# Mourtz/Photorealistic-Rendering-using-OpenCL

Hardware: AMD Instinct MI355X
Metric: Msamples/s (width x height x spp / s) at 1920x1080 (higher is better)
Workload: dtype f32

## Files before the change

photorealistic-rendering-using-opencl_amd/csrc/hip/pt_device.h:

```cpp
#pragma once
#include <hip/hip_runtime.h>

#include "prt_detmath.h"
#include "prt_types.h"
#include "pt_filter.h"
#include "pt_layout.h"

namespace prt {
namespace dev {

#define PT_EPS 1e-5f
#define PT_INF 2e1f
#define PT_PI 3.1415926535897932384626433832795f
#define PT_TWO_PI 6.283185307179586476925286766559f
#define PT_INV_PI 0.3183098861837906715377675267450f
#define PT_INV_TWO_PI 0.1591549430918953357688837633725f
#define PT_INV_FOUR_PI 0.0795774715459476678844418816863f

#ifdef PT_EMU
#define PT_DEV __host__ __device__ __forceinline__
#else
#define PT_DEV __device__ __forceinline__
#endif
#define PT_HD __host__ __device__ __forceinline__

#if defined(__HIP_DEVICE_COMPILE__)
#define PT_WAVE_ANY(p) __builtin_expect(__builtin_amdgcn_ballot_w64(p) != 0ull, 0)
#endif

#ifndef PT_RECIP_STEPS
#define PT_RECIP_STEPS 1
#endif
PT_HD float hw_recip(float x) {
#if defined(__HIP_DEVICE_COMPILE__)
    const unsigned e = (prt_f2u(x) >> 23) & 0xffu;
    float r = __builtin_amdgcn_rcpf(x);
    for (int k = 0; k < PT_RECIP_STEPS; ++k) r = __builtin_fmaf(__builtin_fmaf(-x, r, 1.0f), r, r);
    if (PT_WAVE_ANY(!(e - 2u < 251u))) r = 1.0f / x;
    return r;
#else
    return 1.0f / x;
#endif
}
PT_HD float hw_sqrt(float x) {
#if defined(__HIP_DEVICE_COMPILE__)
    const unsigned e = (prt_f2u(x) >> 23) & 0x1ffu;
    const float r = __builtin_amdgcn_rsqf(x);
    const float s0 = x * r, hh = 0.5f * r;
    float s = __builtin_fmaf(__builtin_fmaf(-s0, s0, x), hh, s0);
    if (PT_WAVE_ANY(!(e - 27u < 200u))) s = __builtin_sqrtf(x);
    return s;
#else
    return __builtin_sqrtf(x);
#endif
}
struct f3 { float x, y, z; };
PT_HD f3 F3(float x, float y, float z) { f3 r; r.x = x; r.y = y; r.z = z; return r; }
PT_HD f3 splat(float s) { return F3(s, s, s); }
PT_HD f3 operator+(f3 a, f3 b) { return F3(a.x + b.x, a.y + b.y, a.z + b.z); }
PT_HD f3 operator-(f3 a, f3 b) { return F3(a.x - b.x, a.y - b.y, a.z - b.z); }
PT_HD f3 operator*(f3 a, f3 b) { return F3(a.x * b.x, a.y * b.y, a.z * b.z); }
PT_HD f3 operator*(f3 a, float s) { return F3(a.x * s, a.y * s, a.z * s); }
PT_HD f3 operator/(f3 a, float s) { return F3(a.x / s, a.y / s, a.z / s); }
PT_HD f3 operator-(f3 a) { return F3(-a.x, -a.y, -a.z); }
PT_HD float dot(f3 a, f3 b) { return a.x * b.x + a.y * b.y + a.z * b.z; }
PT_HD f3 cross(f3 a, f3 b) { return F3(a.y * b.z - a.z * b.y, a.z * b.x - a.x * b.z, a.x * b.y - a.y * b.x); }
PT_HD float length(f3 a) { return hw_sqrt(a.x * a.x + a.y * a.y + a.z * a.z); }
PT_HD f3 normalize(f3 a) { float inv = hw_recip(hw_sqrt(a.x * a.x + a.y * a.y + a.z * a.z)); return F3(a.x * inv, a.y * inv, a.z * inv); }
PT_HD f3 ld3(const float* p) { return F3(p[0], p[1], p[2]); }

#if defined(__HIP_DEVICE_COMPILE__)
#define PT_CONST __attribute__((address_space(4)))
#else
#define PT_CONST
#endif
typedef float pt_vf4 __attribute__((ext_vector_type(4)));
typedef unsigned pt_vu4 __attribute__((ext_vector_type(4)));
template <typename T> PT_HD const PT_CONST pt_vf4* const_vf4(const T* p) { return (const PT_CONST pt_vf4*)p; }
PT_HD unsigned const_u32(const uint32_t* p, unsigned i) { return ((const PT_CONST uint32_t*)p)[i]; }
PT_HD int const_i32(const int32_t* p, unsigned i) { return ((const PT_CONST int32_t*)p)[i]; }
PT_HD float const_f32(const float* p, size_t i) { return ((const PT_CONST float*)p)[i]; }
template <typename T> PT_HD unsigned table_offset(unsigned i) {
    static_assert(sizeof(T) == 64 || sizeof(T) == 48, "NodePair, or a 48-byte record");
    return sizeof(T) == 64 ? pair_offset(i) : rec48_offset(i);
}
template <typename T> PT_HD const float4* table_at(const T* base, unsigned i) { return reinterpret_cast<const float4*>(reinterpret_cast<const char*>(base) + table_offset<T>(i)); }
template <typename T> PT_HD const PT_CONST pt_vf4* const_table_at(const T* base, unsigned i) { return (const PT_CONST pt_vf4*)((const PT_CONST char*)base + table_offset<T>(i)); }
template <typename T> PT_HD const PT_CONST pt_vf4* const_lane_at(const T* base, unsigned i) { return (const PT_CONST pt_vf4*)((const PT_CONST char*)base + i * (unsigned)sizeof(T)); }
PT_HD DevSphere sphere_of(const PT_CONST pt_vf4* q) {
    const pt_vf4 a = q[0];
    DevSphere s;
    s.pos[0] = a.x; s.pos[1] = a.y; s.pos[2] = a.z; s.radius = a.w;
    return s;
}
PT_HD DevSphere const_sphere(const DevSphere* p, unsigned i) { return sphere_of(const_vf4(p + i)); }
PT_HD DevSphere lane_sphere(const DevSphere* p, unsigned i) { return sphere_of(const_lane_at(p, i)); }
PT_HD DevQuad quad_of(const PT_CONST pt_vf4* q) {
    const pt_vf4 a = q[0], b = q[1], c = q[2], d = q[3], e = q[4];
    DevQuad r;
    r.base[0] = a.x; r.base[1] = a.y; r.base[2] = a.z; r.area = a.w;
    r.edge0[0] = b.x; r.edge0[1] = b.y; r.edge0[2] = b.z; r.e0e0 = b.w;
    r.edge1[0] = c.x; r.edge1[1] = c.y; r.edge1[2] = c.z; r.e1e1 = c.w;
    r.normal[0] = d.x; r.normal[1] = d.y; r.normal[2] = d.z; r.u0 = d.w;
    r.anchor[0] = e.x; r.anchor[1] = e.y; r.anchor[2] = e.z; r.u1 = e.w;
    return r;
}
PT_HD DevQuad const_quad(const DevQuad* p, unsigned i) { return quad_of(const_vf4(p + i)); }
PT_HD DevQuad lane_quad(const DevQuad* p, unsigned i) { return quad_of(const_lane_at(p, i)); }
PT_HD DevSdf sdf_of(const PT_CONST pt_vf4* q) {
    const pt_vf4 a = q[0], b = q[1];
    DevSdf r;
    r.pos[0] = a.x; r.pos[1] = a.y; r.pos[2] = a.z; r.type = prt_f2u(a.w);
    r.params[0] = b.x; r.params[1] = b.y; r.params[2] = b.z; r.params[3] = b.w;
    return r;
}
PT_HD DevSdf const_sdf(const DevSdf* p, unsigned i) { return sdf_of(const_vf4(p + i)); }
PT_HD DevSdf lane_sdf(const DevSdf* p, unsigned i) { return sdf_of(const_lane_at(p, i)); }
PT_DEV f3 vexp(f3 a) { return F3(prt_exp(a.x), prt_exp(a.y), prt_exp(a.z)); }
PT_DEV float fmax3(f3 v) { return prt_fmax(prt_fmax(v.x, v.y), v.z); }
PT_DEV float avg3(f3 v) { return (v.x * 1.0f + v.y * 1.0f + v.z * 1.0f) * 0.3333333333333333333333333333333333333333333333f; }

PT_DEV float hw_min(float a, float b) { return __builtin_fminf(a, b); }
PT_DEV float hw_max(float a, float b) { return __builtin_fmaxf(a, b); }

struct Rng { unsigned s0, s1; };
PT_DEV float next1D(Rng& r) {
    r.s0 = 36969u * (r.s0 & 65535u) + (r.s0 >> 16);
    r.s1 = 18000u * (r.s1 & 65535u) + (r.s1 >> 16);
    unsigned ires = (r.s0 << 16) + r.s1;
    return (prt_u2f((ires & 0x007fffffu) | 0x40000000u) - 2.0f) * 0.5f;
}

struct Frame { f3 normal, tangent, bitangent; };
PT_DEV Frame make_frame(f3 n) {
    Frame f;
    float sn = prt_copysign(1.0f, n.z);
    float a = -hw_recip(sn + n.z);
    float b = n.x * n.y * a;
    f.normal = n;
    f.tangent = F3(1.0f + sn * n.x * n.x * a, sn * b, -sn * n.x);
    f.bitangent = F3(b, sn + n.y * n.y * a, -n.y);
    return f;
}
PT_DEV f3 to_local(const Frame& f, f3 p) { return F3(dot(f.tangent, p), dot(f.bitangent, p), dot(f.normal, p)); }
PT_DEV f3 to_global(const Frame& f, f3 p) { return f.tangent * p.x + f.bitangent * p.y + f.normal * p.z; }

struct Ray {
    f3 origin, dir, normal, pos;
    float t;
    bool backside;
    float time;
};

struct Event {
    f3 wi, wo, weight;
    float pdf;
    unsigned sampledLobe;
    Frame frame;
};

struct Mat {
    f3 color, eta, k;
    float roughness;
    unsigned t, lobes, dist;
};
template <unsigned DM = 7u>
PT_DEV Mat load_mat(const DevMaterial* mats, unsigned i) {
    Mat r;
    const PT_CONST pt_vf4* q = const_table_at(mats, i);
    const pt_vf4 a = q[0], e = q[1], kk = q[2];
    r.color = F3(a.x, a.y, a.z); r.roughness = a.w;
    r.eta = F3(e.x, e.y, e.z); r.k = F3(kk.x, kk.y, kk.z);
    unsigned b = prt_f2u(e.w);
    r.t = b & 0xffffu; r.lobes = (b >> 16) & 0xffu; r.dist = (b >> 24) & DM;
    return r;
}

PT_DEV unsigned mat_bits(const DevMaterial* mats, unsigned i) { return *(const PT_CONST uint32_t*)((const PT_CONST char*)mats + (rec48_offset(i) + 28u)); }
PT_DEV unsigned mat_index(int mesh_id) { return (unsigned)(mesh_id + 1) & 0xffffffu; }

PT_DEV void sincos_pair(float x, float& sin_out, float& cos_out) {
    const bool unsupported = !(prt_fabs(x) < 1.0e9f);
    float s, c; int q;
    prt_sincos_kernel(unsupported ? 0.0f : x, &s, &c, &q);
    const float vs = (q & 1) ? c : s, vc = (q & 1) ? s : c;
    const float sn = (q & 2) ? -vs : vs, cs = ((q + 1) & 2) ? -vc : vc;
    const float z = x - x;
    sin_out = unsupported ? z : sn;
    cos_out = unsupported ? z : cs;
}

PT_DEV f3 uniform_sphere(float xi_x, float xi_y) {
    float phi = xi_x * PT_TWO_PI;
    float z = xi_y * 2.0f - 1.0f;
    float r = hw_sqrt(prt_fmax(1.0f - z * z, 0.0f));
    float sn, cs;
    sincos_pair(phi, sn, cs);
    return F3(cs * r, sn * r, z);
}
PT_DEV f3 cosine_hemisphere(float xi_x, float xi_y) {
    float phi = xi_x * PT_TWO_PI;
    float r = hw_sqrt(xi_y);
    float sn, cs;
    sincos_pair(phi, sn, cs);
    return F3(cs * r, sn * r, hw_sqrt(prt_fmax(1.0f - xi_y, 0.0f)));
}
PT_DEV bool check_reflection(f3 wi, f3 wo) {
    return prt_fabs(wi.z * wo.z - wi.x * wo.x - wi.y * wo.y - 1.0f) < 1e-3f;
}
PT_DEV bool check_refraction(f3 wi, f3 wo, float eta, float cosThetaT) {
    float dotP = -wi.x * wo.x * eta - wi.y * wo.y * eta - prt_copysign(cosThetaT, wi.z) * wo.z;
    return prt_fabs(dotP - 1.0f) < 1e-3f;
}

PT_HD void camera_basis(const prt_camera& in, DevCamera& cam) {
    f3 view = normalize(ld3(in.view));
    f3 up = normalize(ld3(in.up));
    f3 hAxis = normalize(cross(view, up));
    f3 vAxis = normalize(cross(hAxis, view));
    f3 position = ld3(in.position);
    f3 middle = position + view;
    f3 horizontal = hAxis * prt_tan(in.fov[0] * 0.5f * (PT_PI / 180));
    f3 vertical = vAxis * prt_tan(in.fov[1] * -0.5f * (PT_PI / 180));
    cam.position[0] = position.x; cam.position[1] = position.y; cam.position[2] = position.z;
    cam.hAxis[0] = hAxis.x; cam.hAxis[1] = hAxis.y; cam.hAxis[2] = hAxis.z;
    cam.vAxis[0] = vAxis.x; cam.vAxis[1] = vAxis.y; cam.vAxis[2] = vAxis.z;
    cam.middle[0] = middle.x; cam.middle[1] = middle.y; cam.middle[2] = middle.z;
    cam.horizontal[0] = horizontal.x; cam.horizontal[1] = horizontal.y; cam.horizontal[2] = horizontal.z;
    cam.vertical[0] = vertical.x; cam.vertical[1] = vertical.y; cam.vertical[2] = vertical.z;
    cam.apertureRadius = in.apertureRadius; cam.focalDistance = in.focalDistance;
}

PT_DEV Ray create_cam_ray(int cx, int cy, int width, int height, const DevCamera& cam, Rng& rng) {
    const f3 hAxis = ld3(cam.hAxis), vAxis = ld3(cam.vAxis), position = ld3(cam.position);
    const f3 middle = ld3(cam.middle), horizontal = ld3(cam.horizontal), vertical = ld3(cam.vertical);
    int pixelx = cx;
    int pixely = height - cy - 1;
    float sx = (float)pixelx / (width - 1.0f);
    float sy = (float)pixely / (height - 1.0f);
    f3 onPlane = middle + (horizontal * ((2 * sx) - 1)) + (vertical * ((2 * sy) - 1));
    f3 onImagePlane = position + ((onPlane - position) * cam.focalDistance);
    f3 aperturePoint;
    if (cam.apertureRadius > 0.00001f) {
        float random1 = next1D(rng);
        float random2 = next1D(rng);
        float angle = 2 * PT_PI * random1;
        float distance = cam.apertureRadius * hw_sqrt(random2);
        float sn, cs;
        sincos_pair(angle, sn, cs);
        float apertureX = cs * distance;
        float apertureY = sn * distance;
        aperturePoint = position + (hAxis * apertureX) + (vAxis * apertureY);
    } else {
        aperturePoint = position;
    }
    Ray ray;
    ray.backside = false;
    ray.origin = aperturePoint;
    ray.dir = normalize(onImagePlane - aperturePoint);
    ray.time = next1D(rng);
    ray.normal = splat(0.0f);
    ray.pos = splat(0.0f);
    ray.t = 0.0f;
    return ray;
}
PT_DEV Ray create_cam_ray_at(int cx, int cy, float dx, float dy, int width, int height, const DevCamera& cam, Rng& rng) {
    const f3 hAxis = ld3(cam.hAxis), vAxis = ld3(cam.vAxis), position = ld3(cam.position);
    const f3 middle = ld3(cam.middle), horizontal = ld3(cam.horizontal), vertical = ld3(cam.vertical);
    const int pixely = height - cy - 1;
    const float sx = ((float)cx + dx) / (width - 1.0f);
    const float sy = ((float)pixely - dy) / (height - 1.0f);
    const f3 onPlane = middle + (horizontal * ((2 * sx) - 1)) + (vertical * ((2 * sy) - 1));
    const f3 onImagePlane = position + ((onPlane - position) * cam.focalDistance);
    f3 aperturePoint;
    if (cam.apertureRadius > 0.00001f) {
        const float random1 = next1D(rng);
        const float random2 = next1D(rng);
        const float angle = 2 * PT_PI * random1;
        const float distance = cam.apertureRadius * hw_sqrt(random2);
        float sn, cs;
        sincos_pair(angle, sn, cs);
        const float apertureX = cs * distance;
        const float apertureY = sn * distance;
        aperturePoint = position + (hAxis * apertureX) + (vAxis * apertureY);
    } else {
        aperturePoint = position;
    }
    Ray ray;
    ray.backside = false;
    ray.origin = aperturePoint;
    ray.dir = normalize(onImagePlane - aperturePoint);
    ray.time = next1D(rng);
    ray.normal = splat(0.0f);
    ray.pos = splat(0.0f);
    ray.t = 0.0f;
    return ray;
}

struct RayPre { float ix, iy, iz, sx, sy, sz; bool nx, ny, nz; };
PT_DEV RayPre ray_pre(const Ray& ray) {
    RayPre p;
    p.ix = hw_recip(ray.dir.x); p.iy = hw_recip(ray.dir.y); p.iz = hw_recip(ray.dir.z);
    p.sx = -ray.origin.x * p.ix; p.sy = -ray.origin.y * p.iy; p.sz = -ray.origin.z * p.iz;
    p.nx = ray.dir.x < 0.0f; p.ny = ray.dir.y < 0.0f; p.nz = ray.dir.z < 0.0f;
    return p;
}

struct TriHit { float u, v; unsigned slot; };

PT_DEV bool hit_triangle_data(const float4 a, const float4 b, const float4 c4, const unsigned slot, const Ray& ray, float& best_t, TriHit& th) {
    const f3 p0 = F3(a.x, a.y, a.z), e1 = F3(a.w, b.x, b.y), e2 = F3(b.z, b.w, c4.x), n = F3(c4.y, c4.z, c4.w);
    f3 c = p0 - ray.origin;
    f3 r = cross(ray.dir, c);
    float inv_det = hw_recip(dot(n, ray.dir));
    float u = dot(r, e2) * inv_det;
    float v = dot(r, e1) * inv_det;
    float w = 1.0f - u - v;
    if (u >= 0 && v >= 0 && w >= 0) {
        float t = dot(n, c) * inv_det;
        if (t > PT_EPS && t < best_t) {
            best_t = t;
            th.u = u; th.v = v; th.slot = slot;
            return true;
        }
    }
    return false;
}
PT_DEV bool hit_triangle(const TriGeom* __restrict__ tg, unsigned slot, const Ray& ray, float& best_t, TriHit& th) {
    const PT_CONST pt_vf4* q = const_vf4(tg + slot);
    const pt_vf4 a = q[0], b = q[1], c4 = q[2];
    return hit_triangle_data(make_float4(a.x, a.y, a.z, a.w), make_float4(b.x, b.y, b.z, b.w), make_float4(c4.x, c4.y, c4.z, c4.w), slot, ray, best_t, th);
}

struct TravStack {
    unsigned* lds;
    unsigned stride;
};

struct PairData { float4 b0, b1, b2; uint4 meta; };
PT_DEV PairData load_pair(const NodePair* __restrict__ pairs, unsigned node) {
    const float4* q = table_at(pairs, node);
    PairData d;
    d.b0 = q[0]; d.b1 = q[1]; d.b2 = q[2];
    d.meta = *reinterpret_cast<const uint4*>(q + 3);
    return d;
}
struct PairTest { float entry0, entry1; bool go0, go1; };
PT_DEV PairTest test_pair(const PairData& d, const RayPre& p, float best_t) {
    const float4 b0 = d.b0, b1 = d.b1, b2 = d.b2;
    PairTest r;
    float e0x = prt_fma(p.nx ? b0.y : b0.x, p.ix, p.sx), x0x = prt_fma(p.nx ? b0.x : b0.y, p.ix, p.sx);
    float e0y = prt_fma(p.ny ? b0.w : b0.z, p.iy, p.sy), x0y = prt_fma(p.ny ? b0.z : b0.w, p.iy, p.sy);
    float e0z = prt_fma(p.nz ? b1.y : b1.x, p.iz, p.sz), x0z = prt_fma(p.nz ? b1.x : b1.y, p.iz, p.sz);
    float e1x = prt_fma(p.nx ? b1.w : b1.z, p.ix, p.sx), x1x = prt_fma(p.nx ? b1.z : b1.w, p.ix, p.sx);
    float e1y = prt_fma(p.ny ? b2.y : b2.x, p.iy, p.sy), x1y = prt_fma(p.ny ? b2.x : b2.y, p.iy, p.sy);
    float e1z = prt_fma(p.nz ? b2.w : b2.z, p.iz, p.sz), x1z = prt_fma(p.nz ? b2.z : b2.w, p.iz, p.sz);
    r.entry0 = hw_max(e0x, hw_max(e0y, hw_max(e0z, PT_EPS)));
    const float exit0 = hw_min(x0x, hw_min(x0y, hw_min(x0z, best_t)));
    r.entry1 = hw_max(e1x, hw_max(e1y, hw_max(e1z, PT_EPS)));
    const float exit1 = hw_min(x1x, hw_min(x1y, hw_min(x1z, best_t)));
    r.go0 = r.entry0 <= exit0;
    r.go1 = r.entry1 <= exit1;
    return r;
}

PT_DEV PairData load_pair_uniform(const NodePair* __restrict__ pairs, unsigned node) {
    const PT_CONST pt_vf4* q = const_vf4(pairs + node);
    const pt_vf4 a = q[0], b = q[1], c = q[2], m = q[3];
    PairData d;
    d.b0 = make_float4(a.x, a.y, a.z, a.w); d.b1 = make_float4(b.x, b.y, b.z, b.w); d.b2 = make_float4(c.x, c.y, c.z, c.w);
    d.meta = make_uint4(prt_f2u(m.x), prt_f2u(m.y), prt_f2u(m.z), prt_f2u(m.w));
    return d;
}
struct TravRes { bool found; float t; TriHit th; };

#if defined(PT_WALK_STATS) && !defined(PT_EMU)
__device__ unsigned long long g_walk_stats[16];
#define PT_WSTAT(k) do { const unsigned long long m_ = __ballot(1); if ((threadIdx.x & 63u) == (unsigned)__builtin_ctzll(m_)) { atomicAdd(&g_walk_stats[2 * (k)], 1ull); atomicAdd(&g_walk_stats[2 * (k) + 1], (unsigned long long)__popcll(m_)); } } while (0)
#else
#define PT_WSTAT(k) do { } while (0)
#endif
struct WalkState {
    unsigned node;
    unsigned sp : 7, pend_count : 25;
    float t, u, v;
    unsigned slot : 29, found : 1, done : 1, last : 1;
    unsigned pend_first;
};

PT_DEV void walk_begin(const DevScene& sc, const bool ANY_HIT, const Ray& ray, const float tmax, const RayPre& p, WalkState& w,
                       const TravStack& stack) {
    w.found = false; w.done = false; w.last = false;
    w.slot = 0;
    w.pend_count = 0; w.pend_first = 0;
    if (!ANY_HIT) { w.t = tmax; w.u = w.v = 0.0f; }
    float t_any = tmax;
    TriHit th;
    th.u = th.v = 0.0f; th.slot = 0;
    w.node = 0; w.sp = 0;
    if (sc.root_is_leaf) {
        for (unsigned i = sc.root_leaf_first; i < sc.root_leaf_first + sc.root_leaf_count; ++i)
            if (hit_triangle(sc.tri_geom, i, ray, ANY_HIT ? t_any : w.t, th)) { w.found = true; if (ANY_HIT) break; w.u = th.u; w.v = th.v; w.slot = th.slot; }
        w.done = true;
        return;
    }
    const PairData d = load_pair_uniform(sc.pairs, 0u);
    const PairTest pt = test_pair(d, p, ANY_HIT ? tmax : w.t);
    const uint4 meta = d.meta;
    if (!((pt.go0 & (meta.y != 0xFFFFFFFFu)) | (pt.go1 & (meta.w != 0xFFFFFFFFu)))) {
        if (pt.go0 != pt.go1) {
            w.node = pt.go0 ? meta.x : meta.z;
        } else if (pt.go0) {
            unsigned nearc = meta.x, farc = meta.z;
            if (pt.entry0 > pt.entry1) { nearc = meta.z; farc = meta.x; }
            stack.lds[0] = farc;
            w.sp = 1;
            w.node = nearc;
        } else {
            w.done = true;
        }
    }
}

PT_DEV void walk_box_data(const PairData& d, const bool ANY_HIT, const Ray& ray, const RayPre& p, WalkState& w, const TravStack& stack) {
    PT_WSTAT(ANY_HIT ? 2 : 0);
    const PairTest pt = test_pair(d, p, ANY_HIT ? ray.t : w.t);
    const uint4 meta = d.meta;
    bool go0 = pt.go0, go1 = pt.go1;
    const bool hit_leaf0 = go0 & (meta.y != 0xFFFFFFFFu), hit_leaf1 = go1 & (meta.w != 0xFFFFFFFFu);
    unsigned pend = 0u;
    if (hit_leaf0 | hit_leaf1) {
        w.pend_first = hit_leaf0 ? meta.x : meta.z;
        pend = (hit_leaf0 ? meta.y : 0u) + (hit_leaf1 ? meta.w : 0u);
        if (hit_leaf0) go0 = false;
        if (hit_leaf1) go1 = false;
    }
    w.pend_count = pend;
    if (go0 != go1) {
        w.node = go0 ? meta.x : meta.z;
    } else if (go0) {
        unsigned nearc = meta.x, farc = meta.z;
        if (pt.entry0 > pt.entry1) { nearc = meta.z; farc = meta.x; }
        stack.lds[w.sp * stack.stride] = farc;
        ++w.sp;
        w.node = nearc;
    } else if (w.sp == 0u) {
        if (pend) w.last = true; else w.done = true;
    } else {
        --w.sp;
        w.node = stack.lds[w.sp * stack.stride];
    }
}

PT_DEV void walk_tri_data(const float4 a, const float4 b, const float4 c4, const bool ANY_HIT, const Ray& ray, WalkState& w) {
    PT_WSTAT(ANY_HIT ? 3 : 1);
    float t_any = ray.t;
    TriHit th;
    th.u = th.v = 0.0f; th.slot = 0;
    const unsigned i = w.pend_first;
    w.pend_first = i + 1u;
    const unsigned left = w.pend_count - 1u;
    w.pend_count = left;
    if (hit_triangle_data(a, b, c4, i, ray, ANY_HIT ? t_any : w.t, th)) {
        w.found = true;
        if (ANY_HIT) { w.pend_count = 0; w.done = true; return; }
        w.u = th.u; w.v = th.v; w.slot = th.slot;
    }
    if (left == 0u && w.last) w.done = true;
}

PT_DEV void walk_box(const DevScene& sc, const bool ANY_HIT, const Ray& ray, const RayPre& p, WalkState& w, const TravStack& stack) {
    const PairData d = load_pair(sc.pairs, w.node);
    walk_box_data(d, ANY_HIT, ray, p, w, stack);
}
PT_DEV void walk_tri(const DevScene& sc, const bool ANY_HIT, const Ray& ray, WalkState& w) {
    const float4* q = table_at(sc.tri_geom, w.pend_first);
    const float4 a = q[0], b = q[1], c4 = q[2];
    walk_tri_data(a, b, c4, ANY_HIT, ray, w);
}
PT_DEV bool hit_sphere(const DevSphere& s, const Ray& ray, float& best_t) {
    f3 p = ray.origin - ld3(s.pos);
    float B = dot(p, ray.dir);
    float C = dot(p, p) - s.radius * s.radius;
    float detSq = B * B - C;
    if (detSq >= 0.0f) {
        float det = hw_sqrt(detSq);
        float t = -B - det;
        if (t < best_t && t > PT_EPS) { best_t = t; return true; }
        t = -B + det;
        if (t < best_t && t > PT_EPS) { best_t = t; return true; }
    }
    return false;
}
PT_DEV bool out_of_unit_range(float x, float c, float u) {
    const bool divide = !(prt_fabs(x) >= 7.888609052210118e-31f) || u != u;
#if defined(__HIP_DEVICE_COMPILE__)
    bool out = x < 0.0f || (x - c) > u;
    if (PT_WAVE_ANY(divide)) {
        const float l = x / c;
        out = l < 0.0f || l > 1.0f;
    }
    return out;
#else
    if (divide) {
        const float l = x / c;
        return l < 0.0f || l > 1.0f;
    }
    return x < 0.0f || (x - c) > u;
#endif
}
PT_DEV bool hit_quad(const DevQuad& qd, const Ray& ray, float& best_t, f3& q_out) {
    const f3 normal = ld3(qd.normal), anchor = ld3(qd.anchor);
    const float nDotW = dot(normal, ray.dir);
    const float rt = dot(normal, anchor - ray.origin) / nDotW;
    if (nDotW <= 1e-5f || rt <= PT_EPS || rt >= best_t) return false;
    f3 q = ray.origin + ray.dir * rt;
    f3 v = q - anchor;
    const float x0 = dot(v, ld3(qd.edge0)), x1 = dot(v, ld3(qd.edge1));
    const bool out0 = out_of_unit_range(x0, qd.e0e0, qd.u0), out1 = out_of_unit_range(x1, qd.e1e1, qd.u1);
    if (out0 || out1) return false;
    best_t = rt;
    q_out = q;
    return true;
}
PT_DEV f3 vabs3(f3 a) { return F3(prt_fabs(a.x), prt_fabs(a.y), prt_fabs(a.z)); }
PT_DEV f3 vmax0(f3 a) { return F3(prt_fmax(a.x, 0.0f), prt_fmax(a.y, 0.0f), prt_fmax(a.z, 0.0f)); }
PT_DEV float s_map(const DevSdf& sdf, f3 pos) {
    const f3 c = pos - ld3(sdf.pos);
    const f3 b = ld3(sdf.params);
    if (sdf.type & (1u << 4)) return length(c) - sdf.params[0];
    else if (sdf.type & (1u << 5)) {
        f3 d = vabs3(c) - b;
        return prt_fmin(prt_fmax(d.x, prt_fmax(d.y, d.z)), 0.0f) + length(vmax0(d));
    } else if (sdf.type & (1u << 6)) return length(vmax0(vabs3(c) - b)) - sdf.params[3];
    else if (sdf.type & (1u << 7)) return dot(c, b) + sdf.params[3];
    return PT_INF;
}
PT_DEV float sdf_map(const DevScene& sc, float tmin, f3 pos, int& id) {
    float dist = tmin;
    for (unsigned i = 0; i < sc.n_sdfs; ++i) {
        const float temp_dist = s_map(const_sdf(sc.sdfs, i), pos);
        if (temp_dist < dist) { dist = temp_dist; id = (int)(sc.n_spheres + i); }
    }
    return dist;
}
PT_DEV f3 sdf_normal(const DevSdf& m, f3 pos) {
    const float e = PT_EPS * 2.0f;
    return normalize(F3(s_map(m, pos + F3(e, 0, 0)) - s_map(m, pos - F3(e, 0, 0)),
                        s_map(m, pos + F3(0, e, 0)) - s_map(m, pos - F3(0, e, 0)),
                        s_map(m, pos + F3(0, 0, e)) - s_map(m, pos - F3(0, 0, e))));
}
PT_DEV bool shadow_sdf(const DevScene& sc, const f3 o, const f3 d, const float tmax) {
    float t = PT_EPS * 100.0f;
    int id = -1;
    for (int i = 0; i < sc.shadow_marching_steps; ++i) {
        const float h = prt_fabs(sdf_map(sc, tmax, o + d * t, id));
        t += h;
        if (h < PT_EPS || t > tmax) break;
    }
    return t <= tmax;
}
PT_DEV bool intersect_sdf(const DevScene& sc, const Ray& ray, float& best_t, int& mesh_id) {
    float t = PT_EPS * 10.0f;
    int id = -1;
    for (int i = 0; i < sc.marching_steps; ++i) {
        const float h = prt_fabs(sdf_map(sc, best_t, ray.origin + ray.dir * t, id));
        if (h < PT_EPS || t > best_t) break;
        t += h;
    }
    if (t > best_t) return false;
    best_t = t;
    mesh_id = id;
    return true;
}

template <bool SDF>
PT_DEV bool finish_closest(const DevScene& sc, Ray& ray, const TravRes& tr, int& mesh_id) {
    float t = tr.t;
    mesh_id = -1;
    if (tr.found) {
        const float4* nq = table_at(sc.tri_nrm, tr.th.slot);
        const float4 a = nq[0], b = nq[1], c = nq[2];
        ray.normal = F3(a.x, a.y, a.z) * (1.0f - tr.th.u - tr.th.v) + F3(b.x, b.y, b.z) * tr.th.u + F3(c.x, c.y, c.z) * tr.th.v;
    }
    ray.normal = normalize(ray.normal);
    ray.pos = ray.origin + ray.dir * t;
// ... 484 lines not shown
template <unsigned MATS>
PT_DEV f3 bsdf_eval2(const DevScene& sc, const Event& e, const Mat& mat) {
    const unsigned am = active_mats<MATS>(sc);
    const unsigned t = mat.t & am;
    f3 f;
    if (t & PRT_MAT_DIFF) f = lambert_eval(e, mat);
    else if (t & PRT_MAT_COND) f = conductor_eval(e, mat);
    else if (t & PRT_MAT_ROUGH_COND) f = rough_conductor_eval(e.wi, e.wo, mat);
    else if (t & PRT_MAT_DIEL) f = dielectric_eval(e, mat);
    else if (t & PRT_MAT_ROUGH_DIEL) f = rough_dielectric_eval(e, mat);
    else if (t & PRT_MAT_COAT) f = coat_eval(e, mat);
    else f = splat(0.0f);
    if (am & (PRT_MAT_DIEL | PRT_MAT_ROUGH_DIEL)) {
        float eta = 1.0f;
        if (t & (PRT_MAT_DIEL | PRT_MAT_ROUGH_DIEL)) eta = dielectric_eta(e, mat);
        f = f * (eta * eta);
    }
    return f;
}
template <unsigned MATS>
PT_DEV float bsdf_pdf(const DevScene& sc, const Event& e, const Mat& mat) {
    const unsigned t = mat.t & active_mats<MATS>(sc);
    if (t & PRT_MAT_DIFF) return 0.0f;
    else if (t & PRT_MAT_COND) return check_reflection(e.wi, e.wo) ? 1.0f : 0.0f;
    else if (t & PRT_MAT_ROUGH_COND) return rough_conductor_pdf(e.wi, e.wo, mat);
    else if (t & PRT_MAT_DIEL) return dielectric_pdf(e, mat);
    else if (t & PRT_MAT_ROUGH_DIEL) return rough_dielectric_pdf(e, mat);
    else if (t & PRT_MAT_COAT) return coat_pdf(e, mat);
    return 0.0f;
}

PT_DEV float hg(float g, float cosTheta) {
    float term = 1.0f + g * g - 2.0f * g * cosTheta;
    return PT_INV_FOUR_PI * (1.0f - g * g) / (term * hw_sqrt(term));
}
PT_DEV float rayleigh(float cosTheta) { return (3.0f / (16.0f * PT_PI)) * (1.0f + cosTheta * cosTheta); }
PT_DEV float phase_value(const DevScene& sc, f3 wi, f3 wo) {
    if (sc.phase_function == 2) return rayleigh(dot(wi, wo));
    if (sc.phase_function == 1) return hg(sc.phase_g, dot(wi, wo));
    return PT_INV_FOUR_PI;
}
struct PhaseSample { f3 w, weight; float pdf; };
PT_DEV void phase_sample(const DevScene& sc, f3 wi, PhaseSample& ps, Rng& rng) {
    float xi_x = next1D(rng), xi_y = next1D(rng);
    ps.weight = splat(1.0f);
    if (sc.phase_function == 2) {
        float phi = xi_x * PT_TWO_PI;
        float z = xi_y * 4.0f - 2.0f;
        float invZ = hw_sqrt(z * z + 1.0f);
        float u = prt_cbrt(z + invZ);
        float cosTheta = u - hw_recip(u);
        float sinTheta = hw_sqrt(prt_fmax(1.0f - cosTheta * cosTheta, 0.0f));
        Frame tf = make_frame(wi);
        float sn, cs;
        sincos_pair(phi, sn, cs);
        ps.w = to_global(tf, F3(cs * sinTheta, sn * sinTheta, cosTheta));
        ps.pdf = rayleigh(cosTheta);
    } else if (sc.phase_function == 1 && sc.phase_g != 0.0f) {
        const float g = sc.phase_g;
        float phi = xi_x * PT_TWO_PI;
        float q = (1.0f - g * g) / (1.0f + g * (xi_y * 2.0f - 1.0f));
        float cosTheta = (1.0f + g * g - q * q) / (2.0f * g);
        float sinTheta = hw_sqrt(prt_fmax(1.0f - cosTheta * cosTheta, 0.0f));
        Frame tf = make_frame(wi);
        float sn, cs;
        sincos_pair(phi, sn, cs);
        ps.w = to_global(tf, F3(cs * sinTheta, sn * sinTheta, cosTheta));
        ps.pdf = hg(g, cosTheta);
    } else {
        ps.w = uniform_sphere(xi_x, xi_y);
        ps.pdf = PT_INV_FOUR_PI;
    }
}
struct MediumSample { f3 p, weight; bool exited; };
PT_DEV void medium_sample_distance(const DevScene& sc, MediumSample& ms, const Ray& ray, Rng& rng) {
    const f3 sigmaT = splat(sc.fog_sigma_t), sigmaS = splat(sc.fog_sigma_s);
    const float maxT = ray.t;
    float mt;
    if (sc.fog_abs_only) {
        mt = maxT;
        ms.weight = vexp(sigmaT * (-mt));
        ms.exited = true;
    } else {
        int lane = (int)prt_round(next1D(rng) * 3.0f);
        float sigmaTc = (lane == 3) ? 0.0f : sc.fog_sigma_t;
        float t = -prt_log(1.0f - next1D(rng)) / sigmaTc;
        mt = prt_fmin(t, maxT);
        ms.exited = (t >= maxT);
        f3 tau = sigmaT * mt;
        ms.weight = vexp(-tau);
        float pdf;
        if (ms.exited) {
            pdf = avg3(vexp(-tau));
        } else {
            pdf = avg3(sigmaT * vexp(-tau));
            ms.weight = ms.weight * sigmaS;
        }
        ms.weight = ms.weight / pdf;
    }
    ms.p = ray.origin + ray.dir * mt;
}

PT_DEV f3 env_texel(const DevScene& sc, int i, int j) {
    if (i < 0 || j < 0 || i >= sc.env_w || j >= sc.env_h) return splat(0.0f);
    const unsigned texel = ((unsigned)j & 0xffffffu) * ((unsigned)sc.env_w & 0xffffffu) + (unsigned)i;
    const float* p = reinterpret_cast<const float*>(reinterpret_cast<const char*>(sc.env) + texel * 12u);
    return F3(p[0], p[1], p[2]);
}
PT_DEV f3 env_lookup(const DevScene& sc, f3 dir) {
    float cx = (prt_atan2(dir.z, dir.x) * PT_INV_TWO_PI) + 0.5f;
    float cy = prt_acos(dir.y) * PT_INV_PI;
    float u = cx * (float)sc.env_w, v = cy * (float)sc.env_h;
    float fu = prt_floor(u - 0.5f), fv = prt_floor(v - 0.5f);
    float a = (u - 0.5f) - fu, b = (v - 0.5f) - fv;
    int i0 = (int)fu, j0 = (int)fv;
    f3 t00 = env_texel(sc, i0, j0), t10 = env_texel(sc, i0 + 1, j0), t01 = env_texel(sc, i0, j0 + 1), t11 = env_texel(sc, i0 + 1, j0 + 1);
    return t00 * ((1.f - a) * (1.f - b)) + t10 * (a * (1.f - b)) + t01 * ((1.f - a) * b) + t11 * (a * b);
}

struct EnvSample { f3 d; float pdf; };
PT_DEV unsigned cdf_find(const float* __restrict__ cdf, unsigned n, float xi) {
    unsigned lo = 0u, hi = n;
    while (hi - lo > 1u) { const unsigned mid = (lo + hi) >> 1; if (cdf[mid] <= xi) lo = mid; else hi = mid; }
    return lo;
}
PT_DEV float env_texel_pdf(const DevScene& sc, unsigned i, unsigned j, float sin_theta) {
    const float* cols = sc.env_cdf_cols + (size_t)j * (unsigned)(sc.env_w + 1);
    const float prow = sc.env_cdf_rows[j + 1u] - sc.env_cdf_rows[j], pcol = cols[i + 1u] - cols[i];
    if (!(sin_theta > 0.0f)) return 0.0f;
    return prow * pcol * (float)sc.env_w * (float)sc.env_h / (2.0f * PT_PI * PT_PI * sin_theta);
}
PT_DEV EnvSample env_sample(const DevScene& sc, float xi0, float xi1) {
    const unsigned j = cdf_find(sc.env_cdf_rows, (unsigned)sc.env_h, xi0);
    const float r0 = sc.env_cdf_rows[j], r1 = sc.env_cdf_rows[j + 1u];
    const float* cols = sc.env_cdf_cols + (size_t)j * (unsigned)(sc.env_w + 1);
    const unsigned i = cdf_find(cols, (unsigned)sc.env_w, xi1);
    const float c0 = cols[i], c1 = cols[i + 1u];
    const float fv = r1 > r0 ? (xi0 - r0) / (r1 - r0) : 0.5f, fu = c1 > c0 ? (xi1 - c0) / (c1 - c0) : 0.5f;
    const float u = ((float)i + fu) / (float)sc.env_w, v = ((float)j + fv) / (float)sc.env_h;
    const float phi = (u - 0.5f) * PT_TWO_PI, theta = v * PT_PI;
    float st, ct, sp, cp;
    sincos_pair(theta, st, ct);
    sincos_pair(phi, sp, cp);
    EnvSample es;
    es.d = F3(st * cp, ct, st * sp);
    es.pdf = env_texel_pdf(sc, i, j, st);
    return es;
}
PT_DEV float env_pdf(const DevScene& sc, f3 dir) {
    const float cx = (prt_atan2(dir.z, dir.x) * PT_INV_TWO_PI) + 0.5f, cy = prt_acos(dir.y) * PT_INV_PI;
    if (!(cx == cx) || !(cy == cy)) return 0.0f;
    int i = (int)(cx * (float)sc.env_w), j = (int)(cy * (float)sc.env_h);
    i = i < 0 ? 0 : (i >= sc.env_w ? sc.env_w - 1 : i);
    j = j < 0 ? 0 : (j >= sc.env_h ? sc.env_h - 1 : j);
    return env_texel_pdf(sc, (unsigned)i, (unsigned)j, prt_sqrt(dir.x * dir.x + dir.z * dir.z));
}
template <unsigned MATS>
PT_DEV float bsdf_pdf_sampling(const DevScene& sc, const Event& e, const Mat& mat) {
    if (mat.t & active_mats<MATS>(sc) & PRT_MAT_DIFF) return (e.wi.z <= 0.0f || e.wo.z <= 0.0f) ? 0.0f : prt_fabs(e.wo.z) * PT_INV_PI;
    return bsdf_pdf<MATS>(sc, e, mat);
}

PT_DEV float power_heuristic(float pdf0, float pdf1) { return (pdf0 * pdf0) / (pdf0 * pdf0 + pdf1 * pdf1); }

struct Hit { float t; f3 normal; int mesh_id : 24; unsigned didHit : 1, backside : 1; };

enum { K_NONE = 0, K_SURFACE_MIS = 1, K_SCATTER = 2 };
enum { ST_READY = 0, ST_WALKC = 1, ST_BACK = 2, ST_WALKS = 3, ST_FINISH = 4 };

struct Lane {
    f3 mask;
    float acc[4];
    unsigned total, samples;
    unsigned diff : 16, spec : 16;
    unsigned trans : 16, scatters : 16;
    f3 origin, dir;
    float t, time;
    Hit h;
    Rng rng;
    f3 weight;
    int mesh_id;
    union {
        struct { f3 wi, n_shade; float pdf; };
        struct {
            f3 vis;
            f3 sh_d;
            float sh_tmax;
        };
    };
    float ps_pdf;
    union {
        WalkState w;
        struct { unsigned w_node_, w_sp_; f3 a; };
    };
    f3 view_n;
    unsigned f;
    unsigned stage : 3;
    unsigned kind : 2;
    unsigned sampledLobe : 8;
    unsigned wasSpecular : 1, reset : 1;
    unsigned h_valid : 1;
    unsigned terminate : 1, w2_ran : 1;
    unsigned sh : 1;
    unsigned begun : 1;
    unsigned fresh : 1;
    unsigned w2 : 1;
    unsigned occluded : 1;
    unsigned sh_vertex : 1;
    unsigned posted : 1;
    unsigned conv : 1;
};

PT_DEV f3 lane_hit_pos(const Lane& L) { return L.origin + L.dir * L.h.t; }

PT_DEV void lane_init(Lane& L) {
    L.kind = K_NONE; L.mesh_id = -1; L.terminate = L.w2_ran = L.sh = false;
    L.weight = L.vis = L.sh_d = splat(0.0f);
    L.sampledLobe = 0u; L.sh_tmax = 0.0f; L.ps_pdf = 1.0f;
    L.rng.s0 = L.rng.s1 = 0u;
    L.h.t = 0.0f; L.h.normal = splat(0.0f); L.h.mesh_id = -1; L.h.didHit = L.h.backside = false; L.h_valid = false;
    L.w.node = 0u; L.w.sp = 0u; L.w.pend_count = 0u; L.w.pend_first = 0u; L.w.t = 0.0f; L.w.u = L.w.v = 0.0f; L.w.slot = 0u; L.w.found = false; L.w.done = true; L.w.last = false;
    L.f = 0u; L.stage = ST_READY;
    L.begun = L.fresh = L.w2 = L.occluded = false;
    L.sh_vertex = false;
    L.posted = false;
}

PT_DEV bool lane_owes_frames(const FrameArgs& fa, const Lane& L, const unsigned target) {
    if (L.stage != ST_READY || L.begun) return L.f < target;
    if (fa.spp_limit && L.reset && L.samples >= fa.spp_limit) return false;
    return L.f < target;
}
PT_DEV bool lane_owes_frames(const FrameArgs& fa, const Lane& L) { return lane_owes_frames(fa, L, fa.n_frames); }
PT_DEV bool lane_runnable(const FrameArgs& fa, const Lane& L, const bool laggards, const unsigned target) {
    if (L.stage != ST_READY) return false;
    if (L.begun) return true;
    if (fa.spp_limit && L.reset && L.samples >= fa.spp_limit) return false;
    return L.f < target || (fa.run_ahead && laggards && L.f < fa.seed_frames);
}
PT_DEV bool lane_frozen_adaptive(const FrameArgs& fa, const Lane& L) { return L.reset && (L.samples >= fa.spp_limit || L.conv); }
PT_DEV bool lane_owes_frames_adaptive(const FrameArgs& fa, const Lane& L, const unsigned target) {
    if (L.stage != ST_READY || L.begun) return L.f < target;
    if (lane_frozen_adaptive(fa, L)) return false;
    return L.f < target;
}
PT_DEV bool lane_runnable_adaptive(const FrameArgs& fa, const Lane& L, const bool laggards, const unsigned target) {
    if (L.stage != ST_READY) return false;
    if (L.begun) return true;
    if (lane_frozen_adaptive(fa, L)) return false;
    return L.f < target || (fa.run_ahead && laggards && L.f < fa.seed_frames);
}
PT_HD bool adaptive_converged(const float l, const float s2, const unsigned n, const float rel_err, const float abs_floor) {
    const float m = l / (float)n;
    const float v = __builtin_fmaxf((s2 - l * m) / ((float)n * (float)(n - 1u)), 0.0f);
    const float t = rel_err * __builtin_fmaxf(m, abs_floor);
    return v < t * t;
}
PT_DEV bool lane_runnable(const FrameArgs& fa, const Lane& L, const bool laggards) { return lane_runnable(fa, L, laggards, fa.n_frames); }

template <unsigned MATS, bool MEDIUM>
PT_DEV void lane_finish_segment(const DevScene& sc, Lane& L, f3 emission, const float alpha, const bool surface, bool done, const bool lit) {
    if (L.kind == K_SURFACE_MIS) {
        const f3 b = lit ? L.vis : splat(0.0f);
        emission = emission + (L.a + b) * L.mask;
    } else if (MEDIUM && L.kind == K_SCATTER) {
        const f3 a = lit ? L.vis : splat(0.0f);
        emission = emission + (a + L.a) * L.mask;
        L.mask = L.mask * L.weight;
    }
    if (surface && !done) {
        L.wasSpecular = (L.sampledLobe & PRT_LOBE_SPECULAR) != 0;
        L.mask = L.mask * L.weight;
        L.diff = (L.diff + ((L.sampledLobe & (PRT_LOBE_DIFFUSE_R | PRT_LOBE_GLOSSY_R)) != 0)) & 0xffffu;
        L.spec = (L.spec + ((L.sampledLobe & PRT_LOBE_SPECULAR_R) != 0)) & 0xffffu;
        L.trans = (L.trans + ((L.sampledLobe & PRT_LOBE_TRANSMISSIVE) != 0)) & 0xffffu;
        if (L.terminate) {
            L.reset = true;
            done = true;
        } else {
            L.scatters = 0;
            ++L.total;
        }
    }
    if (!done) {
        const float roulettePdf = fmax3(L.mask);
        if (L.total > 2 && roulettePdf < 0.1f) {
            if (next1D(L.rng) < roulettePdf) L.mask = L.mask / roulettePdf;
            else { L.reset = true; done = true; }
        }
    }
    if (!done) {
        if (L.total >= (unsigned)sc.max_bounces || (int)L.diff >= sc.max_diff_bounces ||
            (int)L.spec >= sc.max_spec_bounces || (int)L.trans >= sc.max_trans_bounces)
            L.reset = true;
    }
    if (MATS & PT_MATS_VIEW) { L.acc[0] = L.view_n.x; L.acc[1] = L.view_n.y; L.acc[2] = L.view_n.z; L.acc[3] = 1.0f; }
    else { L.acc[0] += emission.x; L.acc[1] += emission.y; L.acc[2] += emission.z; L.acc[3] += alpha; }
    ++L.f;
    L.begun = false;
    L.stage = ST_READY;
}

template <unsigned MATS, bool MEDIUM>
PT_DEV void lane_front(const DevScene& sc, const DevCamera& cam, const FrameArgs& fa, Lane& L, int gx, int gy) {
    if (!L.begun) {
        const unsigned frame = fa.first_frame + L.f;
        const int random0 = const_i32(fa.seed_pairs, 2u * L.f), random1 = const_i32(fa.seed_pairs, 2u * L.f + 1u);
        L.rng.s0 = (unsigned)gx * frame % 1000u + ((unsigned)random0 * 100u);
        L.rng.s1 = (unsigned)gy * frame % 1000u + ((unsigned)random1 * 100u);
        { const float tt = L.t; L.t = L.time; L.time = tt; }
        if (L.reset || L.samples == 0) {
            ++L.samples;
            L.total = 0; L.diff = 0; L.spec = 0; L.trans = 0; L.scatters = 0;
            L.wasSpecular = true;
            L.reset = false;
            L.mask = splat(1.0f);
            L.h_valid = false;
            Ray cr;
            if constexpr ((MATS & PT_MATS_FILTER) != 0u) {
                float dx, dy;
                filter_offset(fa.filter_kind, fa.filter_r, fa.filter_tab, (unsigned)gx, (unsigned)gy, L.samples - 1u, dx, dy);
                cr = create_cam_ray_at(gx, gy, dx, dy, fa.width, fa.full_height, cam, L.rng);
            } else {
                cr = create_cam_ray(gx, gy, fa.width, fa.full_height, cam, L.rng);
            }
            L.origin = cr.origin; L.dir = cr.dir; L.t = cr.t; L.time = cr.time;
        }
        L.begun = true;
    }
    if (!L.h_valid) {
        L.stage = ST_WALKC; L.fresh = true; L.w2 = false;
        return;
    }
    const unsigned am = active_mats<MATS>(sc);
    Ray ray;
    ray.origin = L.origin; ray.dir = L.dir; ray.time = L.time;
    ray.t = L.h.t; ray.normal = L.h.normal; ray.pos = lane_hit_pos(L); ray.backside = L.h.backside;
    if (MATS & PT_MATS_VIEW) L.view_n = L.h.didHit ? ray.normal : normalize(splat(0.0f));
    const bool didHit = L.h.didHit;
    L.mesh_id = L.h.mesh_id;
    L.t = L.h.t;
    L.h_valid = false;
    L.kind = K_NONE; L.terminate = false; L.w2_ran = false; L.sh = false;
    L.vis = splat(0.0f);
    const Mat mat = load_mat<dist_mask<MATS>()>(sc.mats, (L.mesh_id + 1) ? (unsigned)(L.mesh_id + 1) : sc.n_meshes + 1u);
    f3 emission = splat(0.0f);
    float alpha = 1.0f;
    if (MEDIUM) {
        MediumSample ms;
        medium_sample_distance(sc, ms, ray, L.rng);
        L.mask = L.mask * ms.weight;
        if (!ms.exited && (int)L.scatters < sc.max_scattering_events) {
            L.kind = K_SCATTER;
            L.scatters = (L.scatters + 1u) & 0xffffu;
            L.wasSpecular = false;
            LightSample rec;
            unsigned lmesh;
            if (sample_light(sc, (MATS & PT_MATS_PICK) != 0, ray.pos, rec, L.rng, lmesh)) {
                const float fv = phase_value(sc, ray.dir, rec.d);
                const f3 f = splat(fv);
                if (!(dot(f, f) == 0.0f)) {
                    L.sh = true; L.sh_d = rec.d; L.sh_tmax = rec.dist;
                    const Mat lm = load_mat(sc.mats, lmesh + 1u);
                    const f3 tr = vexp(splat(sc.fog_sigma_t) * (-1.0f * rec.dist));
                    const f3 contribution = tr * lm.color * f * power_heuristic(rec.pdf, fv);
                    L.vis = contribution / rec.pdf;
                }
            }
            PhaseSample ps;
            phase_sample(sc, ray.dir, ps, L.rng);
            L.origin = ms.p; L.dir = ps.w; L.weight = ps.weight; L.ps_pdf = ps.pdf;
            L.w2_ran = true;
            L.stage = ST_WALKC; L.fresh = true; L.w2 = true;
            return;
        }
    }
    if (!didHit) {
        L.reset = true;
        if (sc.alpha_testing) { emission = splat(0.0f); alpha = 0.0f; }
        else emission = L.mask * env_lookup(sc, ray.dir);
        lane_finish_segment<MATS, MEDIUM>(sc, L, emission, alpha, false, true, false);
        return;
    }
    if ((am & PRT_MAT_LIGHT) && (mat.t & PRT_MAT_LIGHT)) {
        if (L.wasSpecular) emission = emission + mat.color * L.mask;
        L.reset = true;
        lane_finish_segment<MATS, MEDIUM>(sc, L, emission, alpha, false, true, false);
        return;
    }
    Event e;
    e.wo = splat(0.0f); e.weight = splat(1.0f); e.pdf = 1.0f; e.sampledLobe = 0;
    e.frame = make_frame(ray.normal);
    e.wi = to_local(e.frame, -ray.dir);
    const bool mis = (am & PRT_MAT_LIGHT) && (mat.lobes & ~(PRT_LOBE_SPECULAR | PRT_LOBE_FORWARD) & 0xffu);
    const bool ok = bsdf_sample2<MATS>(sc, e, ray, mat, L.rng);
    L.wi = e.wi; L.weight = e.weight; L.pdf = e.pdf; L.sampledLobe = e.sampledLobe; L.n_shade = ray.normal;
    if (ok) {
        L.origin = ray.pos;
        L.dir = to_global(e.frame, e.wo);
    }
    if (mis) {
        L.kind = K_SURFACE_MIS;
        if (ok) { L.w2_ran = true; L.stage = ST_WALKC; L.fresh = true; L.w2 = true; }
        else { L.terminate = true; L.stage = ST_BACK; }
    } else if (ok) {
        lane_finish_segment<MATS, MEDIUM>(sc, L, emission, alpha, true, false, false);
    } else {
        L.reset = true;
        lane_finish_segment<MATS, MEDIUM>(sc, L, emission, alpha, false, true, false);
    }
}

template <bool MEDIUM>
PT_DEV Ray lane_closest_ray(const Lane& L) {
    Ray r;
    r.pos = splat(0.0f); r.backside = false; r.t = PT_INF; r.time = 0.0f;
    if (MEDIUM && L.w2 && L.kind == K_SCATTER) {
        r.origin = L.origin; r.dir = L.dir; r.normal = splat(0.0f);
    } else {
        r.origin = L.origin; r.dir = L.dir;
        r.normal = L.w2 ? L.h.normal : splat(0.0f);
    }
    return r;
}

template <unsigned MATS, bool MEDIUM>
PT_DEV void lane_closest_done(const DevScene& sc, Lane& L) {
    TravRes r;
    r.found = L.w.found; r.t = L.w.t; r.th.u = L.w.u; r.th.v = L.w.v; r.th.slot = L.w.slot;
    Ray wr = lane_closest_ray<MEDIUM>(L);
    int mid;
    const bool hit = finish_closest<(MATS & PT_MATS_SDF) != 0>(sc, wr, r, mid);
    L.h.t = wr.t; L.h.normal = wr.normal; L.h.mesh_id = mid; L.h.didHit = hit; L.h.backside = wr.backside;
    L.h_valid = true;
    if ((MATS & PT_MATS_VIEW) && L.w2 && !(MEDIUM && L.kind == K_SCATTER)) L.view_n = wr.normal;
    if (!L.w2) {
        L.stage = ST_READY;
    } else {
        if (!(MEDIUM && L.kind == K_SCATTER)) L.t = wr.t;
        L.stage = ST_BACK;
    }
}

template <unsigned MATS, bool MEDIUM>
PT_DEV void lane_back(const DevScene& sc, Lane& L) {
    const f3 hit_pos = lane_hit_pos(L);
    L.a = splat(0.0f);
    f3 sh_o = hit_pos;
    if (MATS & PT_MATS_ENVIS) L.sh_vertex = false;
    if (L.kind == K_SURFACE_MIS) {
        constexpr bool ENVIS = (MATS & PT_MATS_ENVIS) != 0;
        const Mat mat = load_mat<dist_mask<MATS>()>(sc.mats, (L.mesh_id + 1) ? (unsigned)(L.mesh_id + 1) : sc.n_meshes + 1u);
        bool env_live = false;
        if (ENVIS) {
            const unsigned lobe = L.w2_ran ? L.sampledLobe : mat.lobes;
            const int diff = (int)L.diff + ((lobe & (PRT_LOBE_DIFFUSE_R | PRT_LOBE_GLOSSY_R)) != 0), spec = (int)L.spec + ((lobe & PRT_LOBE_SPECULAR_R) != 0);
            const int trans = (int)L.trans + ((lobe & PRT_LOBE_TRANSMISSIVE) != 0);
            env_live = !(L.total + 1u >= (unsigned)sc.max_bounces || diff >= sc.max_diff_bounces || spec >= sc.max_spec_bounces || trans >= sc.max_trans_bounces);
        }
        if (L.w2_ran && L.h.didHit) {
            const int mid = L.h.mesh_id;
            const unsigned lbits = mat_bits(sc.mats, (unsigned)(mid + 1));
            if (lbits & PRT_MAT_LIGHT) {
                const Mat lm = load_mat(sc.mats, (unsigned)(mid + 1));
                L.a = lm.color * L.weight * power_heuristic(L.pdf, direct_pdf_mesh(sc, mid, L.dir, hit_pos));
                if (MEDIUM) L.a = L.a * vexp(splat(sc.fog_sigma_t) * (-1.0f * L.t));
            }
        } else if (ENVIS && L.w2_ran) {
            L.terminate = true;
            float keep = env_live ? 1.0f : 0.0f;
            const float roulettePdf = fmax3(L.mask * L.weight);
            if (env_live && L.total + 1u > 2u && roulettePdf < 0.1f) keep = next1D(L.rng) < roulettePdf ? 1.0f / roulettePdf : 0.0f;
            if (keep > 0.0f) {
                const float w = (L.sampledLobe & PRT_LOBE_SPECULAR) ? 1.0f : power_heuristic(L.pdf, 0.5f * env_pdf(sc, L.dir));
                L.a = env_lookup(sc, L.dir) * L.weight * (w * keep);
            }
        }
        if (ENVIS && env_live && next1D(L.rng) < 0.5f) {
            const float xi0 = next1D(L.rng), xi1 = next1D(L.rng);
            const EnvSample es = env_sample(sc, xi0, xi1);
            if (es.pdf > 0.0f) {
                Event e;
                e.frame = make_frame(L.n_shade);
                e.wi = L.wi; e.weight = L.weight; e.pdf = L.pdf; e.sampledLobe = L.sampledLobe;
                e.wo = to_local(e.frame, es.d);
                const f3 fr = bsdf_eval2<MATS>(sc, e, mat);
                if (!(dot(fr, fr) == 0.0f)) {
                    if (L.w2_ran) { sh_o = L.origin; L.sh_vertex = true; }
                    L.sh = true; L.sh_d = es.d; L.sh_tmax = PT_INF;
                    const float pe = 0.5f * es.pdf;
                    L.vis = env_lookup(sc, es.d) * fr * (power_heuristic(pe, bsdf_pdf_sampling<MATS>(sc, e, mat)) / pe);
                }
            }
        } else {
            LightSample rec;
            unsigned lmesh;
            if (sample_light(sc, (MATS & PT_MATS_PICK) != 0, hit_pos, rec, L.rng, lmesh)) {
                Event e;
                e.frame = make_frame(L.n_shade);
                e.wi = L.wi; e.weight = L.weight; e.pdf = L.pdf; e.sampledLobe = L.sampledLobe;
                e.wo = to_local(e.frame, rec.d);
                const f3 fr = bsdf_eval2<MATS>(sc, e, mat);
                if (!(dot(fr, fr) == 0.0f)) {
                    L.sh = true; L.sh_d = rec.d; L.sh_tmax = rec.dist;
                    const Mat lm = load_mat(sc.mats, lmesh + 1u);
                    f3 contribution = lm.color * fr;
                    if (MEDIUM) contribution = contribution * vexp(splat(sc.fog_sigma_t) * (-1.0f * rec.dist));
                    contribution = contribution * power_heuristic(rec.pdf, bsdf_pdf<MATS>(sc, e, mat));
                    L.vis = contribution / rec.pdf;
                    if (ENVIS && env_live) L.vis = L.vis * 2.0f;
                }
            }
        }
    } else if (MEDIUM && L.kind == K_SCATTER) {
        sh_o = L.origin;
        if (L.h.didHit) {
            const int mid = L.h.mesh_id;
            const unsigned lbits = mat_bits(sc.mats, (unsigned)(mid + 1));
            if (lbits & PRT_MAT_LIGHT) {
                const Mat lm = load_mat(sc.mats, (unsigned)(mid + 1));
                const f3 tr = vexp(splat(sc.fog_sigma_t) * (-1.0f * L.h.t));
                L.a = tr * lm.color * L.weight * power_heuristic(L.ps_pdf, direct_pdf_mesh(sc, mid, L.dir, L.origin));
            }
        }
    }
    if (L.sh && !finish_shadow<(MATS & PT_MATS_SDF) != 0>(sc, sh_o, L.sh_d, L.sh_tmax)) L.sh = false;
    if (L.sh) { L.stage = ST_WALKS; L.fresh = true; }
    else { L.stage = ST_FINISH; L.occluded = false; }
}

template <bool MEDIUM, bool ENVIS = false>
PT_DEV Ray lane_shadow_ray(const Lane& L) {
    Ray r;
    r.origin = ((MEDIUM && L.kind == K_SCATTER) || (ENVIS && L.sh_vertex)) ? L.origin : lane_hit_pos(L);
    r.dir = L.sh_d; r.normal = splat(0.0f); r.pos = splat(0.0f); r.t = L.sh_tmax; r.backside = false; r.time = 0.0f;
    return r;
}

template <unsigned MATS, bool MEDIUM>
PT_DEV void lane_finish(const DevScene& sc, Lane& L) {
    lane_finish_segment<MATS, MEDIUM>(sc, L, splat(0.0f), 1.0f, L.kind == K_SURFACE_MIS, false, L.sh && !L.occluded);
}

}
}
```

Baseline: 2342.

## Add specialized Lambert-only front path sharing disk sample between camera and BSDF

Adds a specialized lane_front for scenes with only diffuse and light materials and no filter or medium. It draws a single disk sample per step, used either for the lens aperture on restart or for cosine-weighted diffuse sampling, and inlines the Lambert BSDF sampling. In lane_back the material reload is skipped and the Lambert eval is computed directly from the stored weight. This cuts material loads, generic BSDF dispatch and RNG calls, but changes the RNG consumption order, which alters the sample sequence, and it assumes the Lambert path matches the generic one.

```diff
diff --git a/photorealistic-rendering-using-opencl_amd/csrc/hip/pt_device.h b/photorealistic-rendering-using-opencl_amd/csrc/hip/pt_device.h
--- a/photorealistic-rendering-using-opencl_amd/csrc/hip/pt_device.h
+++ b/photorealistic-rendering-using-opencl_amd/csrc/hip/pt_device.h
@@ -282,6 +282,43 @@
         sincos_pair(angle, sn, cs);
         const float apertureX = cs * distance;
         const float apertureY = sn * distance;
+        aperturePoint = position + (hAxis * apertureX) + (vAxis * apertureY);
+    } else {
+        aperturePoint = position;
+    }
+    Ray ray;
+    ray.backside = false;
+    ray.origin = aperturePoint;
+    ray.dir = normalize(onImagePlane - aperturePoint);
+    ray.time = next1D(rng);
+    ray.normal = splat(0.0f);
+    ray.pos = splat(0.0f);
+    ray.t = 0.0f;
+    return ray;
+}
+struct DiskSample { float sn, cs, r, xi2; };
+PT_DEV DiskSample disk_sample(Rng& rng) {
+    DiskSample d;
+    const float xi1 = next1D(rng);
+    d.xi2 = next1D(rng);
+    sincos_pair(xi1 * PT_TWO_PI, d.sn, d.cs);
+    d.r = hw_sqrt(d.xi2);
+    return d;
+}
+PT_DEV Ray cam_ray_from_disk(int cx, int cy, int width, int height, const DevCamera& cam, const bool lens, const DiskSample& ds, Rng& rng) {
+    const f3 hAxis = ld3(cam.hAxis), vAxis = ld3(cam.vAxis), position = ld3(cam.position);
+    const f3 middle = ld3(cam.middle), horizontal = ld3(cam.horizontal), vertical = ld3(cam.vertical);
+    int pixelx = cx;
+    int pixely = height - cy - 1;
+    float sx = (float)pixelx / (width - 1.0f);
+    float sy = (float)pixely / (height - 1.0f);
+    f3 onPlane = middle + (horizontal * ((2 * sx) - 1)) + (vertical * ((2 * sy) - 1));
+    f3 onImagePlane = position + ((onPlane - position) * cam.focalDistance);
+    f3 aperturePoint;
+    if (lens) {
+        float distance = cam.apertureRadius * ds.r;
+        float apertureX = ds.cs * distance;
+        float apertureY = ds.sn * distance;
         aperturePoint = position + (hAxis * apertureX) + (vAxis * apertureY);
     } else {
         aperturePoint = position;
@@ -1372,7 +1409,102 @@
 }
 
 template <unsigned MATS, bool MEDIUM>
+PT_HD constexpr bool lambert_only() { return !MEDIUM && (MATS & ~(PT_MATS_ADAPT | PT_MATS_FILTER)) == (PRT_MAT_LIGHT | PRT_MAT_DIFF); }
+template <unsigned MATS, bool MEDIUM>
+PT_HD constexpr bool shared_disk() { return lambert_only<MATS, MEDIUM>() && !(MATS & PT_MATS_FILTER); }
+
+template <unsigned MATS>
+PT_DEV void lane_front_shared_disk(const DevScene& sc, const DevCamera& cam, const FrameArgs& fa, Lane& L, int gx, int gy) {
+    bool restart = false;
+    if (!L.begun) {
+        const unsigned frame = fa.first_frame + L.f;
+        const int random0 = const_i32(fa.seed_pairs, 2u * L.f), random1 = const_i32(fa.seed_pairs, 2u * L.f + 1u);
+        L.rng.s0 = (unsigned)gx * frame % 1000u + ((unsigned)random0 * 100u);
+        L.rng.s1 = (unsigned)gy * frame % 1000u + ((unsigned)random1 * 100u);
+        { const float tt = L.t; L.t = L.time; L.time = tt; }
+        if (L.reset || L.samples == 0) {
+            ++L.samples;
+            L.total = 0; L.diff = 0; L.spec = 0; L.trans = 0; L.scatters = 0;
+            L.wasSpecular = true;
+            L.reset = false;
+            L.mask = splat(1.0f);
+            L.h_valid = false;
+            restart = true;
+        }
+        L.begun = true;
+    }
+    const bool shade = L.h_valid;
+    bool sample = false, mis = false;
+    Frame frame;
+    f3 wi, color;
+    if (shade) {
+        const bool didHit = L.h.didHit;
+        L.mesh_id = L.h.mesh_id;
+        L.t = L.h.t;
+        L.h_valid = false;
+        L.kind = K_NONE; L.terminate = false; L.w2_ran = false; L.sh = false;
+        L.vis = splat(0.0f);
+        const Mat mat = load_mat<dist_mask<MATS>()>(sc.mats, (L.mesh_id + 1) ? (unsigned)(L.mesh_id + 1) : sc.n_meshes + 1u);
+        if (!didHit) {
+            f3 emission = splat(0.0f);
+            float alpha = 1.0f;
+            L.reset = true;
+            if (sc.alpha_testing) alpha = 0.0f;
+            else emission = L.mask * env_lookup(sc, L.dir);
+            lane_finish_segment<MATS, false>(sc, L, emission, alpha, false, true, false);
+        } else if (mat.t & PRT_MAT_LIGHT) {
+            f3 emission = splat(0.0f);
+            if (L.wasSpecular) emission = emission + mat.color * L.mask;
+            L.reset = true;
+            lane_finish_segment<MATS, false>(sc, L, emission, 1.0f, false, true, false);
+        } else {
+            frame = make_frame(L.h.normal);
+            wi = to_local(frame, -L.dir);
+            color = mat.color;
+            mis = (mat.lobes & ~(PRT_LOBE_SPECULAR | PRT_LOBE_FORWARD) & 0xffu) != 0u;
+            sample = (mat.t & PRT_MAT_DIFF) && !(wi.z <= 0.0f);
+            if (!sample) {
+                L.wi = wi; L.weight = splat(1.0f); L.pdf = 1.0f; L.sampledLobe = 0u; L.n_shade = L.h.normal;
+                if (mis) {
+                    L.kind = K_SURFACE_MIS; L.terminate = true; L.stage = ST_BACK;
+                } else {
+                    L.reset = true;
+                    lane_finish_segment<MATS, false>(sc, L, splat(0.0f), 1.0f, false, true, false);
+                }
+            }
+        }
+    }
+    const bool lens = cam.apertureRadius > 0.00001f;
+    const bool need_disk = sample || (restart && lens);
+    DiskSample ds;
+    if (need_disk) ds = disk_sample(L.rng);
+    if (restart) {
+        const Ray cr = cam_ray_from_disk(gx, gy, fa.width, fa.full_height, cam, lens, ds, L.rng);
+        L.origin = cr.origin; L.dir = cr.dir; L.t = cr.t; L.time = cr.time;
+    }
+    if (sample) {
+        const f3 wo = F3(ds.cs * ds.r, ds.sn * ds.r, hw_sqrt(prt_fmax(1.0f - ds.xi2, 0.0f)));
+        L.wi = wi; L.weight = color; L.pdf = prt_fabs(wo.z) * PT_INV_PI; L.sampledLobe = PRT_LOBE_DIFFUSE_R; L.n_shade = L.h.normal;
+        L.origin = lane_hit_pos(L);
+        L.dir = to_global(frame, wo);
+        if (mis) {
+            L.kind = K_SURFACE_MIS;
+            L.w2_ran = true; L.stage = ST_WALKC; L.fresh = true; L.w2 = true;
+        } else {
+            lane_finish_segment<MATS, false>(sc, L, splat(0.0f), 1.0f, true, false, false);
+        }
+    }
+    if (!shade) {
+        L.stage = ST_WALKC; L.fresh = true; L.w2 = false;
+    }
+}
+
+template <unsigned MATS, bool MEDIUM>
 PT_DEV void lane_front(const DevScene& sc, const DevCamera& cam, const FrameArgs& fa, Lane& L, int gx, int gy) {
+    if constexpr (shared_disk<MATS, MEDIUM>()) {
+        lane_front_shared_disk<MATS>(sc, cam, fa, L, gx, gy);
+        return;
+    }
     if (!L.begun) {
         const unsigned frame = fa.first_frame + L.f;
         const int random0 = const_i32(fa.seed_pairs, 2u * L.f), random1 = const_i32(fa.seed_pairs, 2u * L.f + 1u);
@@ -1520,7 +1652,8 @@
     if (MATS & PT_MATS_ENVIS) L.sh_vertex = false;
     if (L.kind == K_SURFACE_MIS) {
         constexpr bool ENVIS = (MATS & PT_MATS_ENVIS) != 0;
-        const Mat mat = load_mat<dist_mask<MATS>()>(sc.mats, (L.mesh_id + 1) ? (unsigned)(L.mesh_id + 1) : sc.n_meshes + 1u);
+        constexpr bool REUSE = lambert_only<MATS, MEDIUM>();
+        const Mat mat = REUSE ? Mat() : load_mat<dist_mask<MATS>()>(sc.mats, (L.mesh_id + 1) ? (unsigned)(L.mesh_id + 1) : sc.n_meshes + 1u);
         bool env_live = false;
         if (ENVIS) {
             const unsigned lobe = L.w2_ran ? L.sampledLobe : mat.lobes;
@@ -1570,7 +1703,9 @@
                 e.frame = make_frame(L.n_shade);
                 e.wi = L.wi; e.weight = L.weight; e.pdf = L.pdf; e.sampledLobe = L.sampledLobe;
                 e.wo = to_local(e.frame, rec.d);
-                const f3 fr = bsdf_eval2<MATS>(sc, e, mat);
+                f3 fr;
+                if (REUSE) fr = (L.w2_ran && !(e.wo.z <= 0.0f)) ? L.weight * PT_INV_PI * e.wo.z : splat(0.0f);
+                else fr = bsdf_eval2<MATS>(sc, e, mat);
                 if (!(dot(fr, fr) == 0.0f)) {
                     L.sh = true; L.sh_d = rec.d; L.sh_tmax = rec.dist;
                     const Mat lm = load_mat(sc.mats, lmesh + 1u);
```

Measured after the change: 2390 (median of 6 runs). 2.1% higher.
